# RemcoHoger/Space-Filling-Curves-for-Vision-Transformers

Hardware: AMD Instinct MI355X
Metric: images/sec ViT-B/16 224px Hilbert-order training (higher is better)
Workload: dtype bf16; 1 GPU; vit_b16_224_hilbert: 224x224 Hilbert pixel order, 16x16-pixel tokens, batch 256/GPU, full train step (fwd+CE+bwd+clip+AdamW); global_batch=256, parallelism=dp1, hip_graph=False

## Files before the change

### space-filling-curves-for-vision-transformers_amd/csrc/gemm8p.hip

```cpp
#include "common_host.h"
#include "gemm_core.h"
#include <mutex>
#include <type_traits>
#include <unordered_map>

namespace sfcvit {
namespace {

using namespace gemm_core;

namespace p8 {

constexpr int T = 512, HALF = 16384, KTB = 65536, LDS_BYTES = 2 * KTB;
constexpr int LDS_TQ = LDS_BYTES, LDS_PATCH = LDS_TQ + 64, LDS_BIAS = LDS_PATCH + 8 * 2048, LDS_MAX = P8_LDS_MAX;
static_assert(LDS_BIAS == P8_LDS_BIAS, "dispatch.h prices the bias vector at this offset");
enum { RELU = P8_RELU, DROP = P8_DROP, RES = P8_RES, DACT = P8_DACT, CSUM = P8_CSUM, BITS = P8_BITS };

typedef const __attribute__((address_space(1))) void *gptr_t;
typedef __attribute__((address_space(3))) void *lptr_t;

template <int N> __device__ __forceinline__ void wait_vm() { asm volatile("s_waitcnt vmcnt(%0)" ::"n"(N) : "memory"); }
template <int N> __device__ __forceinline__ void wait_lgkm() {
    asm volatile("s_waitcnt lgkmcnt(%0)" ::"n"(N) : "memory");
    __builtin_amdgcn_sched_barrier(0);
}
__device__ __forceinline__ void bar() {
    __builtin_amdgcn_sched_barrier(0);
    __builtin_amdgcn_s_barrier();
    __builtin_amdgcn_sched_barrier(0);
}

struct Cursor {
    int tile, k0;
    const uint16_t *p;
};

struct StoreMap {
    int wa;
    int ra;
    long coff;
};

template <int MASK>
__device__ __forceinline__ void epilogue_math(const sfcvit_gemm_args &g, int m, int n, float (&v)[16], const float (&bv)[16],
                                              const u32x4 (&side)[2], uint32_t thresh, float keep_scale, float dact_scale,
                                              uint32_t rk_in0, uint32_t rk_in1, u32x4 &w0, u32x4 &w1) {
    if (!(MASK & DACT)) {
#pragma unroll
        for (int r = 0; r < 16; r++) v[r] += bv[r];
    }
    if (MASK & RELU) {
#pragma unroll
        for (int r = 0; r < 16; r++) v[r] = fmaxf(v[r], 0.f);
    }
    if (MASK & DROP) {
        const uint64_t row = uint64_t(m) + uint64_t(uint32_t(g.row_offset));
        const uint32_t rk = mix32(uint32_t(row) * 0x9E3779B1u + ((row >> 32) ? rk_in1 : rk_in0));
#pragma unroll
        for (int p = 0; p < 8; p++) {
            bool k0, k1;
            drop_keep2(rk, uint32_t(n >> 1) + p, thresh, k0, k1);
            v[2 * p] = k0 ? v[2 * p] * keep_scale : 0.f;
            v[2 * p + 1] = k1 ? v[2 * p + 1] * keep_scale : 0.f;
        }
    }
    if (MASK & RES) {
        float rv[16];
        unpack8f(side[0], rv);
        unpack8f(side[1], rv + 8);
#pragma unroll
        for (int r = 0; r < 16; r++) v[r] += rv[r];
    }
    if ((MASK & BITS) && (MASK & RELU)) {
        uint32_t bits = 0;
#pragma unroll
        for (int r = 0; r < 16; r++) bits |= uint32_t(v[r] > 0.f) << r;
        uint8_t *mp = static_cast<uint8_t *>(g.actmask) + size_t(m) * g.ld_actmask + (n >> 3);
        asm volatile("global_store_short %0, %1, off\n\ts_nop 1" ::"v"(mp), "v"(bits) : "memory");
    }
    if (MASK & DACT) {
        if (MASK & BITS) {
            const uint32_t bits = side[0][0];
#pragma unroll
            for (int r = 0; r < 16; r++) v[r] = (bits >> r & 1u) ? v[r] * dact_scale : 0.f;
        } else {
            float a[16];
            unpack8f(side[0], a);
            unpack8f(side[1], a + 8);
#pragma unroll
            for (int r = 0; r < 16; r++) v[r] = a[r] > 0.f ? v[r] * dact_scale : 0.f;
        }
    }
    w0 = u32x4{pack2bf(v[0], v[1]), pack2bf(v[2], v[3]), pack2bf(v[4], v[5]), pack2bf(v[6], v[7])};
    w1 = u32x4{pack2bf(v[8], v[9]), pack2bf(v[10], v[11]), pack2bf(v[12], v[13]), pack2bf(v[14], v[15])};
}

#define SFCVIT_XROW(a, b) "ds_write_b128 %[wa], " a "\n\tds_write_b128 %[wb], " b "\n\tds_read_b128 " a ", %[ra]\n\tds_read_b128 " b ", %[ra] offset:1024\n\t"
template <int NR>
__device__ __forceinline__ void patch_exchange(u32x4 (&w)[NR][2], const StoreMap &sm) {
    static_assert(NR >= 1 && NR <= 8, "rows per batch");
    const int wa = sm.wa, wb = sm.wa ^ 16, ra = sm.ra;
    if constexpr (NR == 8)
        asm volatile(SFCVIT_XROW("%0", "%1") SFCVIT_XROW("%2", "%3") SFCVIT_XROW("%4", "%5") SFCVIT_XROW("%6", "%7")
                     SFCVIT_XROW("%8", "%9") SFCVIT_XROW("%10", "%11") SFCVIT_XROW("%12", "%13") SFCVIT_XROW("%14", "%15") "s_waitcnt lgkmcnt(0)"
                     : "+v"(w[0][0]), "+v"(w[0][1]), "+v"(w[1][0]), "+v"(w[1][1]), "+v"(w[2][0]), "+v"(w[2][1]), "+v"(w[3][0]), "+v"(w[3][1]),
                       "+v"(w[4][0]), "+v"(w[4][1]), "+v"(w[5][0]), "+v"(w[5][1]), "+v"(w[6][0]), "+v"(w[6][1]), "+v"(w[7][0]), "+v"(w[7][1])
                     : [wa] "v"(wa), [wb] "v"(wb), [ra] "v"(ra) : "memory");
    else if constexpr (NR == 7)
        asm volatile(SFCVIT_XROW("%0", "%1") SFCVIT_XROW("%2", "%3") SFCVIT_XROW("%4", "%5") SFCVIT_XROW("%6", "%7")
                     SFCVIT_XROW("%8", "%9") SFCVIT_XROW("%10", "%11") SFCVIT_XROW("%12", "%13") "s_waitcnt lgkmcnt(0)"
                     : "+v"(w[0][0]), "+v"(w[0][1]), "+v"(w[1][0]), "+v"(w[1][1]), "+v"(w[2][0]), "+v"(w[2][1]), "+v"(w[3][0]), "+v"(w[3][1]),
                       "+v"(w[4][0]), "+v"(w[4][1]), "+v"(w[5][0]), "+v"(w[5][1]), "+v"(w[6][0]), "+v"(w[6][1])
                     : [wa] "v"(wa), [wb] "v"(wb), [ra] "v"(ra) : "memory");
    else if constexpr (NR == 6)
        asm volatile(SFCVIT_XROW("%0", "%1") SFCVIT_XROW("%2", "%3") SFCVIT_XROW("%4", "%5") SFCVIT_XROW("%6", "%7")
                     SFCVIT_XROW("%8", "%9") SFCVIT_XROW("%10", "%11") "s_waitcnt lgkmcnt(0)"
                     : "+v"(w[0][0]), "+v"(w[0][1]), "+v"(w[1][0]), "+v"(w[1][1]), "+v"(w[2][0]), "+v"(w[2][1]), "+v"(w[3][0]), "+v"(w[3][1]),
                       "+v"(w[4][0]), "+v"(w[4][1]), "+v"(w[5][0]), "+v"(w[5][1])
                     : [wa] "v"(wa), [wb] "v"(wb), [ra] "v"(ra) : "memory");
    else if constexpr (NR == 4)
        asm volatile(SFCVIT_XROW("%0", "%1") SFCVIT_XROW("%2", "%3") SFCVIT_XROW("%4", "%5") SFCVIT_XROW("%6", "%7") "s_waitcnt lgkmcnt(0)"
                     : "+v"(w[0][0]), "+v"(w[0][1]), "+v"(w[1][0]), "+v"(w[1][1]), "+v"(w[2][0]), "+v"(w[2][1]), "+v"(w[3][0]), "+v"(w[3][1])
                     : [wa] "v"(wa), [wb] "v"(wb), [ra] "v"(ra) : "memory");
    else
        static_assert(NR == 8, "patch_exchange: batch sizes 4, 6, 7, 8");
}
#undef SFCVIT_XROW

__device__ __forceinline__ void store_row_pair(const sfcvit_gemm_args &g, int m, int n, const StoreMap &sm, const u32x4 &w0, const u32x4 &w1) {
    uint16_t *c = static_cast<uint16_t *>(g.c) + size_t(m) * g.ldc + n + sm.coff;
    asm volatile("global_store_dwordx4 %0, %1, off sc0 sc1 nt\n\ts_nop 1" ::"v"(c), "v"(w0) : "memory");
    asm volatile("global_store_dwordx4 %0, %1, off sc0 sc1 nt\n\ts_nop 1" ::"v"(c + size_t(8) * g.ldc), "v"(w1) : "memory");
}


template <int NI, int MASK, bool P2 = false>
__global__ __launch_bounds__(T) void gemm8p_kernel(const sfcvit_gemm_args g, unsigned *__restrict__ counters, int stag_slots, int stag_ticks, int walk) {
    constexpr int BM = 32 * NI, GR = 16 * NI;
    extern __shared__ __attribute__((aligned(16))) char smem[];
    if (stag_ticks > 0) {
        const uint64_t until = __builtin_amdgcn_s_memrealtime() + uint64_t((blockIdx.x >> 3) % stag_slots) * uint64_t(stag_ticks);
        while (__builtin_amdgcn_s_memrealtime() < until) __builtin_amdgcn_s_sleep(8);
    }
    const int tid = threadIdx.x, lane = tid & 63, wid = __builtin_amdgcn_readfirstlane(tid >> 6), wr = wid >> 2, wc = wid & 3;
    const int q = lane >> 4, nl = lane & 15;
    const int K = g.K, NT = g.N / 256, ntiles = ((g.M + BM - 1) / BM) * NT, KT = K / 64, m_last = g.M - BM;
    const uint16_t *A = static_cast<const uint16_t *>(g.a);
    const uint16_t *B = static_cast<const uint16_t *>(g.b);
    const int G = gridDim.x, per_xcd = G >> 3, xcd = blockIdx.x & 7;
    int *const tq = reinterpret_cast<int *>(smem + LDS_TQ);
    auto tile_of = [&](unsigned l) __attribute__((always_inline)) {
        const long t = long(l / unsigned(per_xcd)) * G + xcd * per_xcd + int(l % unsigned(per_xcd));
        if (t >= ntiles) return -1;
        if (walk > 0 && walk < NT) {
            const unsigned MT = unsigned(ntiles / NT), full = unsigned(NT / walk) * MT * unsigned(walk), ut = unsigned(t);
            const unsigned wcur = ut < full ? unsigned(walk) : unsigned(NT % walk), base = ut < full ? (ut / (MT * walk)) * walk : unsigned(NT / walk) * walk;
            const unsigned tt = ut < full ? ut % (MT * walk) : ut - full;
            return int((tt / wcur) << 16 | (base + tt % wcur));
        }
        return int((unsigned(t) / unsigned(NT)) << 16 | (unsigned(t) % unsigned(NT)));
    };
    auto finish = [&]() __attribute__((always_inline)) {
        if (tid == 0) {
            const unsigned old = atomicAdd(counters + 8, 1u);
            if (old == unsigned(G) - 1u) {
#pragma unroll
                for (int i = 0; i < 9; i++) counters[i] = 0u;
            }
        }
    };
    if (tid == 0) {
        const unsigned l0 = atomicAdd(counters + xcd, 1u);
        tq[0] = tile_of(l0);
        const unsigned l1 = atomicAdd(counters + xcd, 1u);
        tq[1] = tile_of(l1);
    }
    const bool has_bias = !(MASK & DACT) && g.bias != nullptr;
    if (has_bias)
        for (int i = tid; i < g.N / 8; i += T)
            *reinterpret_cast<u32x4 *>(smem + LDS_BIAS + i * 16) = static_cast<const u32x4 *>(g.bias)[i];
    __syncthreads();

    int tile_cur = __builtin_amdgcn_readfirstlane(tq[0]);
    if (tile_cur < 0) { finish(); return; }
    unsigned drawn = 0;
    if (tid == 0) drawn = atomicAdd(counters + xcd, 1u);
    const int tile_first = tile_cur;
    int t = 0;

    const int r1 = 8 * wid + (lane >> 3);
    const int sc = (lane & 7) ^ ((r1 >> 1) & 7);
    const int w1 = (r1 < GR - 64) ? r1 : r1 - (NI == 7 ? 16 : 32);
    const int b_row = (r1 >> 5) * 64 + ((r1 & 15) >> 2) * 16 + ((r1 >> 4) & 1) * 4 + (r1 & 3);
    const uint32_t voffA0 = (uint32_t(r1) * uint32_t(g.lda) + sc * 8) * 2, voffA1 = (uint32_t(64 + w1) * uint32_t(g.lda) + sc * 8) * 2;
    const uint32_t voffB = (uint32_t(b_row) * uint32_t(g.ldb) + sc * 8) * 2;
    const size_t a_second = size_t(GR) * g.lda, b_second = size_t(128) * g.ldb, b_h1 = size_t(8) * g.ldb;

    auto cursor_at = [&](int seq, int tile, bool is_a) __attribute__((always_inline)) {
        Cursor c;
        c.tile = seq;
        c.k0 = 0;
        if (tile < 0) tile = tile_first;
        c.p = is_a ? A + size_t(min((tile >> 16) * BM, m_last)) * g.lda : B + size_t(tile & 0xFFFF) * 256 * g.ldb;
        return c;
    };
    const uint16_t *next_a = nullptr, *next_b = nullptr;
    auto set_next = [&](int seq) __attribute__((always_inline)) {
        const Cursor na = cursor_at(seq, __builtin_amdgcn_readfirstlane(tq[seq & 3]), true);
        const Cursor nb = cursor_at(seq, __builtin_amdgcn_readfirstlane(tq[seq & 3]), false);
        next_a = na.p;
        next_b = nb.p;
    };
    auto advance = [&](Cursor &c, bool is_a) __attribute__((always_inline)) {
        if (c.k0 + 64 == K) { c.tile++; c.k0 = 0; c.p = is_a ? next_a : next_b; }
        else { c.k0 += 64; c.p += 64; }
    };
    const int m0_wave = wid * 1024;
    auto dma16 = [&](const uint16_t *base, uint32_t voff, int lds) __attribute__((always_inline)) {
        asm volatile("s_mov_b32 m0, %2\n\ts_nop 0\n\tglobal_load_lds_dwordx4 %0, %1"
                     :
                     : "v"(voff), "s"(base), "s"(lds)
                     : "memory");
    };
    auto stage_a = [&](const Cursor &c, int buf, int h) __attribute__((always_inline)) {
        const int d = m0_wave + buf * KTB + h * HALF;
        const uint32_t vo = h ? voffA1 : voffA0;
        dma16(c.p, vo, d);
        dma16(c.p + a_second, vo, d + 8192);
    };
    auto stage_b = [&](const Cursor &c, int buf, int h) __attribute__((always_inline)) {
        const uint16_t *p = c.p + (h ? b_h1 : 0);
        const int d = m0_wave + buf * KTB + 2 * HALF + h * HALF;
        dma16(p, voffB, d);
        dma16(p + b_second, voffB, d + 8192);
    };

    const int o0 = nl * 128 + ((q ^ ((nl >> 1) & 7)) << 4);
    const int a_off0 = wr * 8192 + o0, a_off1 = wr * 8192 + (o0 ^ 64);
    const int b_off0 = 2 * HALF + wc * 4096 + o0, b_off1 = 2 * HALF + wc * 4096 + (o0 ^ 64);
    bf16x8 fa0[4][2], fa1[NI - 4][2], fb0[2][2], fb1[2][2];
    auto read_a0 = [&](int buf) __attribute__((always_inline)) {
#pragma unroll
        for (int i = 0; i < 4; i++) {
            fa0[i][0] = *reinterpret_cast<const bf16x8 *>(smem + a_off0 + buf * KTB + i * 2048);
            fa0[i][1] = *reinterpret_cast<const bf16x8 *>(smem + a_off1 + buf * KTB + i * 2048);
        }
    };
    auto read_a1 = [&](int buf) __attribute__((always_inline)) {
#pragma unroll
        for (int i = 0; i < NI - 4; i++) {
            fa1[i][0] = *reinterpret_cast<const bf16x8 *>(smem + a_off0 + buf * KTB + HALF + i * 2048);
            fa1[i][1] = *reinterpret_cast<const bf16x8 *>(smem + a_off1 + buf * KTB + HALF + i * 2048);
        }
    };
    auto read_b = [&](bf16x8 (&fb)[2][2], int buf, int sub) __attribute__((always_inline)) {
#pragma unroll
        for (int j = 0; j < 2; j++) {
            fb[j][0] = *reinterpret_cast<const bf16x8 *>(smem + b_off0 + buf * KTB + sub * HALF + j * 2048);
            fb[j][1] = *reinterpret_cast<const bf16x8 *>(smem + b_off1 + buf * KTB + sub * HALF + j * 2048);
        }
    };

    f32x4 acc[NI][4];
    auto zero_acc = [&]() __attribute__((always_inline)) {
#pragma unroll
        for (int i = 0; i < NI; i++)
#pragma unroll
            for (int j = 0; j < 4; j++) acc[i][j] = f32x4{0.f, 0.f, 0.f, 0.f};
    };
    auto mma0 = [&](const bf16x8 (&fb)[2][2], int bsub) __attribute__((always_inline)) {
        __builtin_amdgcn_s_setprio(1);
#pragma unroll
        for (int kk = 0; kk < 2; kk++)
#pragma unroll
            for (int i = 0; i < 4; i++)
#pragma unroll
                for (int j = 0; j < 2; j++)
                    acc[i][bsub * 2 + j] = __builtin_amdgcn_mfma_f32_16x16x32_bf16(fb[j][kk], fa0[i][kk], acc[i][bsub * 2 + j], 0, 0, 0);
        __builtin_amdgcn_s_setprio(0);
    };
    auto mma1 = [&](const bf16x8 (&fb)[2][2], int bsub) __attribute__((always_inline)) {
        __builtin_amdgcn_s_setprio(1);
#pragma unroll
        for (int kk = 0; kk < 2; kk++)
#pragma unroll
            for (int i = 0; i < NI - 4; i++)
#pragma unroll
                for (int j = 0; j < 2; j++)
                    acc[4 + i][bsub * 2 + j] = __builtin_amdgcn_mfma_f32_16x16x32_bf16(fb[j][kk], fa1[i][kk], acc[4 + i][bsub * 2 + j], 0, 0, 0);
        __builtin_amdgcn_s_setprio(0);
    };

    const uint32_t thresh = (MASK & DROP) ? drop_thresh(g.dropout_p) : 0u;
    const float keep_scale = (MASK & DROP) ? 1.f / (1.f - g.dropout_p) : 1.f;
    const uint32_t seed_e = (MASK & DROP) ? eff_seed(g.dropout_seed, g.seed_off) : 0u;
    const uint32_t rk_in0 = (MASK & DROP) ? mix32(seed_e) : 0u, rk_in1 = (MASK & DROP) ? mix32(seed_e ^ 0x7FEB352Du) : 0u;
    const float dact_scale = g.dact_scale != 0.f ? g.dact_scale : 1.f;
    auto draw = [&]() __attribute__((always_inline)) {
        if (tid == 0) {
            tq[(t + 2) & 3] = tile_of(drawn);
            drawn = atomicAdd(counters + xcd, 1u);
        }
    };
    auto epilogue = [&]() __attribute__((always_inline)) {
        const int tile = tile_cur;
        int te = tid;
        asm volatile("" : "+v"(te));
        const int le = te & 63, qe = le >> 4, ne = le & 15;
        StoreMap sm;
        {
            const int patch = LDS_PATCH + wid * 2048, r0 = le >> 3, ch = le & 7;
            sm.wa = patch + ne * 128 + (((2 * qe) ^ (ne & 7)) << 4);
            sm.ra = patch + r0 * 128 + ((ch ^ r0) << 4);
            sm.coff = long(r0 - ne) * g.ldc + (8 * ch - 16 * qe);
        }
        const int m_new = (tile >> 16) * BM;
        const int m0 = min(m_new, m_last) + wr * GR + ne, n0 = (tile & 0xFFFF) * 256 + wc * 64 + qe * 16;
        mfma_fence();
        float bv[16];
        if (has_bias) {
            const char *bp = smem + LDS_BIAS + n0 * 2;
            unpack8f(*reinterpret_cast<const u32x4 *>(bp), bv);
            unpack8f(*reinterpret_cast<const u32x4 *>(bp + 16), bv + 8);
        } else {
#pragma unroll
            for (int r = 0; r < 16; r++) bv[r] = 0.f;
        }
        const uint16_t *sp = (MASK & RES) ? static_cast<const uint16_t *>(g.residual) : static_cast<const uint16_t *>(g.aux_in);
        const size_t ld_side = (MASK & RES) ? size_t(g.ldr) : size_t(g.ldaux);
        float cs[16];
#pragma unroll
        for (int r = 0; r < 16; r++) cs[r] = 0.f;
        auto batch = [&](auto i0c, auto i1c) __attribute__((always_inline)) {
            constexpr int i0 = decltype(i0c)::value, i1 = decltype(i1c)::value;
            u32x4 side[i1 - i0][2];
            if ((MASK & DACT) && (MASK & BITS)) {
#pragma unroll
                for (int i = i0; i < i1; i++)
                    side[i - i0][0][0] = *reinterpret_cast<const uint16_t *>(static_cast<const uint8_t *>(g.actmask) +
                                                                             size_t(m0 + 16 * i) * g.ld_actmask + (n0 >> 3));
            } else if (MASK & (RES | DACT)) {
#pragma unroll
                for (int i = i0; i < i1; i++) {
                    const uint16_t *p = sp + size_t(m0 + 16 * i) * ld_side + n0;
                    side[i - i0][0] = *reinterpret_cast<const u32x4 *>(p);
                    side[i - i0][1] = *reinterpret_cast<const u32x4 *>(p + 8);
                }
            }
            u32x4 pk[i1 - i0][2];
            static_for<i0, i1>([&](auto ic) __attribute__((always_inline)) {
                constexpr int i = decltype(ic)::value;
                float v[16] = {acc[i][0][0], acc[i][0][1], acc[i][0][2], acc[i][0][3], acc[i][1][0], acc[i][1][1],
                               acc[i][1][2], acc[i][1][3], acc[i][2][0], acc[i][2][1], acc[i][2][2], acc[i][2][3],
                               acc[i][3][0], acc[i][3][1], acc[i][3][2], acc[i][3][3]};
                epilogue_math<MASK>(g, m0 + 16 * i, n0, v, bv, side[i - i0], thresh, keep_scale, dact_scale, rk_in0, rk_in1,
                                    pk[i - i0][0], pk[i - i0][1]);
                if (MASK & CSUM) {
                    const bool own = m0 + 16 * i >= m_new;
#pragma unroll
                    for (int r = 0; r < 16; r++) cs[r] += own ? v[r] : 0.f;
                }
            });
            patch_exchange<i1 - i0>(pk, sm);
            static_for<i0, i1>([&](auto ic) __attribute__((always_inline)) {
                constexpr int i = decltype(ic)::value;
                store_row_pair(g, m0 + 16 * i, n0, sm, pk[i - i0][0], pk[i - i0][1]);
            });
        };
        if constexpr (NI == 8 && ((MASK & (DROP | RES)) == (DROP | RES) || (MASK & (DACT | CSUM | BITS)) == (DACT | CSUM))) {
            batch(std::integral_constant<int, 0>{}, std::integral_constant<int, 4>{});
            batch(std::integral_constant<int, 4>{}, std::integral_constant<int, NI>{});
        } else {
            batch(std::integral_constant<int, 0>{}, std::integral_constant<int, NI>{});
        }
        if (MASK & CSUM) {
#pragma unroll
            for (int r = 0; r < 16; r++) cs[r] = row16_sum(cs[r]);
            if (ne == 0) {
                float *pp = static_cast<float *>(g.workspace) + size_t(2 * (tile >> 16) + wr) * g.N + n0;
#pragma unroll
                for (int r4 = 0; r4 < 4; r4++)
                    *reinterpret_cast<f32x4 *>(pp + 4 * r4) = f32x4{cs[4 * r4], cs[4 * r4 + 1], cs[4 * r4 + 2], cs[4 * r4 + 3]};
            }
        }
        zero_acc();
    };

    Cursor ca = cursor_at(0, tile_cur, true), cb = cursor_at(0, tile_cur, false);
    stage_b(cb, 0, 0); stage_a(ca, 0, 0); stage_a(ca, 0, 1); stage_b(cb, 0, 1);
    advance(ca, true);
    advance(cb, false);
    if (P2) {
        stage_b(cb, 1, 0); stage_a(ca, 1, 0); stage_b(cb, 1, 1);
        advance(cb, false);
        wait_vm<6>();
    } else {
        stage_b(cb, 1, 0); stage_a(ca, 1, 0); stage_a(ca, 1, 1); stage_b(cb, 1, 1);
        advance(ca, true);
        advance(cb, false);
        wait_vm<8>();
    }
    bar();
    if (wr == 1) bar();
    zero_acc();

    constexpr int NSTORE = 2 * NI + ((MASK & CSUM) ? 4 : 0) + (((MASK & BITS) && (MASK & RELU)) ? NI : 0);
    auto stage_next = [&](int buf) __attribute__((always_inline)) {
        stage_a(ca, buf, 1);
        advance(ca, true);
        stage_b(cb, buf, 1);
        advance(cb, false);
        __builtin_amdgcn_sched_barrier(0);
    };
    auto ktile = [&](int buf, bool first, bool last) __attribute__((always_inline)) {
        read_b(fb0, buf, 0);
        read_a0(buf);
        bar();
        wait_lgkm<0>();
        mma0(fb0, 0);
        bar();
        read_a1(buf);
        bar();
        wait_lgkm<0>();
        mma1(fb0, 0);
        if (first) set_next(t + 1);
        bar();
        read_b(fb1, buf, 1);
        stage_b(cb, buf, 0);
        bar();
        wait_lgkm<0>();
        mma1(fb1, 1);
        bar();
        stage_a(ca, buf, 0);
        if (first && t > 0) wait_vm<4 + NSTORE>();
        else wait_vm<4>();
        bar();
        mma0(fb1, 1);
        if (last) {
            if (wr == 0) {
                bar();
                draw();
            }
            stage_next(buf);
            epilogue();
            if (wr == 1) bar();
        } else {
            bar();
            stage_next(buf);
        }
    };
    auto ktile2 = [&](int buf, bool first, bool last) __attribute__((always_inline)) {
        read_b(fb0, buf, 0);
        read_b(fb1, buf, 1);
        read_a0(buf);
        stage_a(ca, buf ^ 1, 1);
        advance(ca, true);
        __builtin_amdgcn_sched_barrier(0);
        if (first && t > 0) wait_vm<8 + NSTORE>();
        else wait_vm<8>();
        wait_lgkm<0>();
        bar();
        mma0(fb0, 0);
        mma0(fb1, 1);
        if (first) set_next(t + 1);
        bar();
        read_a1(buf);
        stage_b(cb, buf, 0);
        stage_a(ca, buf, 0);
        stage_b(cb, buf, 1);
        advance(cb, false);
        __builtin_amdgcn_sched_barrier(0);
        if (first && t > 0) wait_vm<8 + NSTORE>();
        else wait_vm<8>();
        wait_lgkm<0>();
        bar();
        mma1(fb0, 0);
        mma1(fb1, 1);
        if (last) {
            if (wr == 0) {
                bar();
                draw();
            }
            epilogue();
            if (wr == 1) bar();
        } else {
            bar();
        }
    };
    int kt = 0;
    for (;;) {
        if (P2) ktile2(0, kt == 0, false);
        else ktile(0, kt == 0, false);
        kt += 2;
        const bool last = kt == KT;
        if (P2) ktile2(1, false, last);
        else ktile(1, false, last);
        if (last) {
            kt = 0;
            t++;
            tile_cur = __builtin_amdgcn_readfirstlane(tq[t & 3]);
            if (tile_cur < 0) break;
        }
    }
    if (wr == 0) bar();
    wait_vm<0>();
    finish();
}


template <bool P2>
__global__ __launch_bounds__(T) void gemm8p_km_kernel(const sfcvit_gemm_args g, int kt_per_split, int nsplits) {
    extern __shared__ __attribute__((aligned(16))) char smem[];
    const int tid = threadIdx.x, lane = tid & 63, wid = tid >> 6, wr = wid >> 2, wc = wid & 3;
    const int q4 = lane >> 4, nl = lane & 15;
    const int NT = g.N / 256, KT = g.K / 64;
    const int tiles = (g.M / 256) * NT;
    const int unit = (blockIdx.x & 7) * (gridDim.x >> 3) + (blockIdx.x >> 3);
    if (unit >= tiles * nsplits) return;
    const int tile = unit % tiles, z = unit / tiles;
    const int m0 = (tile / NT) * 256, n0 = (tile % NT) * 256;
    const int kt_beg = z * kt_per_split;
    const int nkt = min(kt_per_split, KT - kt_beg);
    const uint16_t *A = static_cast<const uint16_t *>(g.a) + size_t(kt_beg) * 64 * g.lda + m0;
    const uint16_t *B = static_cast<const uint16_t *>(g.b) + size_t(kt_beg) * 64 * g.ldb + n0;

    const int kr = 4 * wid + (lane >> 4);
    const int sw = (kr & 3) | (((kr >> 3) & 1) << 2);
    const int c16 = ((((lane & 15) >> 1) ^ sw) << 1) | (lane & 1);
    const size_t offA = size_t(kr) * g.lda + c16 * 8, offB = size_t(kr) * g.ldb + c16 * 8;
    const size_t a32 = size_t(32) * g.lda, b32 = size_t(32) * g.ldb, a64 = size_t(64) * g.lda, b64 = size_t(64) * g.ldb;
    char *const lds_piece = smem + tid * 16;
    const uint16_t *ca = A, *cb = B;
    int akt = 0, bkt = 0;
    auto advance_a = [&]() __attribute__((always_inline)) {
        if (++akt < nkt) ca += a64;
    };
    auto advance_b = [&]() __attribute__((always_inline)) {
        if (++bkt < nkt) cb += b64;
    };
    auto stage_a = [&](int buf, int h) __attribute__((always_inline)) {
        const uint16_t *p = ca + offA + h * 128;
        char *d = lds_piece + buf * KTB + h * HALF;
        __builtin_amdgcn_global_load_lds((gptr_t)p, (lptr_t)d, 16, 0, 0);
        __builtin_amdgcn_global_load_lds((gptr_t)(p + a32), (lptr_t)(d + 8192), 16, 0, 0);
    };
    auto stage_b = [&](int buf, int h) __attribute__((always_inline)) {
        const uint16_t *p = cb + offB + h * 128;
        char *d = lds_piece + buf * KTB + 2 * HALF + h * HALF;
        __builtin_amdgcn_global_load_lds((gptr_t)p, (lptr_t)d, 16, 0, 0);
        __builtin_amdgcn_global_load_lds((gptr_t)(p + b32), (lptr_t)(d + 8192), 16, 0, 0);
    };

    const int qq = nl >> 2, pp = nl & 3;
    const int lane_sw = qq | ((q4 & 1) << 2);
    const int row_off = (8 * q4 + qq) * 256 + 8 * pp;
    int a_addr[8], b_addr[4];
#pragma unroll
    for (int i = 0; i < 8; i++)
        a_addr[i] = (i >> 2) * HALF + row_off + (((wr * 4 + (i & 3)) ^ lane_sw) << 5);
#pragma unroll
    for (int j = 0; j < 4; j++)
        b_addr[j] = 2 * HALF + (j >> 1) * HALF + row_off + (((wc * 2 + (j & 1)) ^ lane_sw) << 5);
#define SFCVIT_TR(dst, addr, off) asm volatile("ds_read_b64_tr_b16 %0, %1 offset:" #off : "=v"(dst) : "v"(addr) : "memory")
    auto tr_frag2 = [&](bf16x8 (&f)[2], int addr) __attribute__((always_inline)) {
        bf16x4 l0, h0, l1, h1;
        SFCVIT_TR(l0, addr, 0);
        SFCVIT_TR(h0, addr, 1024);
        SFCVIT_TR(l1, addr, 8192);
        SFCVIT_TR(h1, addr, 9216);
        f[0] = __builtin_shufflevector(l0, h0, 0, 1, 2, 3, 4, 5, 6, 7);
        f[1] = __builtin_shufflevector(l1, h1, 0, 1, 2, 3, 4, 5, 6, 7);
    };
    bf16x8 fa0[4][2], fa1[4][2], fb0[2][2], fb1[2][2];
    auto read_a2 = [&](bf16x8 (&fa)[4][2], int sub, int i0) __attribute__((always_inline)) {
#pragma unroll
        for (int i = i0; i < i0 + 2; i++) tr_frag2(fa[i], a_addr[sub * 4 + i]);
    };
    auto read_b = [&](bf16x8 (&fb)[2][2], int sub) __attribute__((always_inline)) {
#pragma unroll
        for (int j = 0; j < 2; j++) tr_frag2(fb[j], b_addr[sub * 2 + j]);
    };
    auto flip = [&]() __attribute__((always_inline)) {
#pragma unroll
        for (int i = 0; i < 8; i++) a_addr[i] ^= KTB;
#pragma unroll
        for (int j = 0; j < 4; j++) b_addr[j] ^= KTB;
    };

    f32x4 acc[8][4];
#pragma unroll
    for (int i = 0; i < 8; i++)
#pragma unroll
        for (int j = 0; j < 4; j++) acc[i][j] = f32x4{0.f, 0.f, 0.f, 0.f};
    auto mma = [&](const bf16x8 (&fa)[4][2], const bf16x8 (&fb)[2][2], int asub, int bsub) __attribute__((always_inline)) {
        __builtin_amdgcn_s_setprio(1);
#pragma unroll
        for (int kk = 0; kk < 2; kk++)
#pragma unroll
            for (int i = 0; i < 4; i++)
#pragma unroll
                for (int j = 0; j < 2; j++)
                    acc[asub * 4 + i][bsub * 2 + j] =
                        __builtin_amdgcn_mfma_f32_16x16x32_bf16(fb[j][kk], fa[i][kk], acc[asub * 4 + i][bsub * 2 + j], 0, 0, 0);
        __builtin_amdgcn_s_setprio(0);
    };

    if (P2) {
        stage_b(0, 0); stage_a(0, 0); stage_a(0, 1); stage_b(0, 1);
        advance_a();
        advance_b();
        stage_b(1, 0); stage_a(1, 0); stage_b(1, 1);
        advance_b();
        wait_vm<6>();
        bar();
        if (wr == 1) bar();
        auto ktile2 = [&](int buf) __attribute__((always_inline)) {
            read_b(fb0, 0);
            read_b(fb1, 1);
            read_a2(fa0, 0, 0);
            read_a2(fa0, 0, 2);
            stage_a(buf ^ 1, 1);
            advance_a();
            wait_vm<8>();
            wait_lgkm<0>();
            bar();
            mma(fa0, fb0, 0, 0);
            mma(fa0, fb1, 0, 1);
            bar();
            read_a2(fa1, 1, 0);
            read_a2(fa1, 1, 2);
            stage_b(buf, 0);
            stage_a(buf, 0);
            stage_b(buf, 1);
            advance_b();
            wait_vm<8>();
            wait_lgkm<0>();
            bar();
            mma(fa1, fb0, 1, 0);
            mma(fa1, fb1, 1, 1);
            bar();
            flip();
        };
        for (int k = 0; k < nkt; k += 2) {
            ktile2(0);
            ktile2(1);
        }
    } else {
        stage_b(0, 0); stage_a(0, 0); stage_a(0, 1); stage_b(0, 1);
        advance_a();
        advance_b();
        stage_b(1, 0); stage_a(1, 0);
        wait_vm<4>();
        bar();
        if (wr == 1) bar();
        auto ktile = [&](int buf) __attribute__((always_inline)) {
            read_b(fb0, 0);
            read_a2(fa0, 0, 0);
            read_a2(fa0, 0, 2);
            stage_a(buf ^ 1, 1);
            advance_a();
            bar();
            wait_lgkm<0>();
            mma(fa0, fb0, 0, 0);
            bar();
            read_a2(fa1, 1, 0);
            read_a2(fa1, 1, 2);
            stage_b(buf ^ 1, 1);
            advance_b();
            bar();
            wait_lgkm<0>();
            mma(fa1, fb0, 1, 0);
            bar();
            read_b(fb1, 1);
            stage_b(buf, 0);
            bar();
            wait_lgkm<0>();
            mma(fa1, fb1, 1, 1);
            bar();
            stage_a(buf, 0);
            wait_vm<4>();
            bar();
            mma(fa0, fb1, 0, 1);
            bar();
            flip();
        };
        for (int k = 0; k < nkt; k += 2) {
            ktile(0);
            ktile(1);
        }
}
    if (wr == 0) bar();
    wait_vm<0>();
    mfma_fence();
    float *slab = static_cast<float *>(g.workspace) + size_t(z) * g.M * g.N + size_t(m0 + wr * 64 + nl) * g.N + n0 + wc * 32 + 4 * q4;
#pragma unroll
    for (int i = 0; i < 8; i++)
#pragma unroll
        for (int j = 0; j < 4; j++)
            *reinterpret_cast<f32x4 *>(slab + size_t((i >> 2) * 128 + (i & 3) * 16) * g.N + (j >> 1) * 128 + (j & 1) * 16) = acc[i][j];
}

struct DeviceState {
    unsigned *pool = nullptr;
    int next = 0;
    std::unordered_map<hipStream_t, unsigned *> per_stream;
};
constexpr int MAX_DEVICES = 64, SLOTS = 1024, SLOT_UINTS = 16;
std::mutex g_mu;
DeviceState g_dev[MAX_DEVICES];

unsigned *queue_counters(hipStream_t s) {
    std::lock_guard<std::mutex> lock(g_mu);
    int dev = 0;
    if (hipGetDevice(&dev) != hipSuccess || dev < 0 || dev >= MAX_DEVICES) return nullptr;
    DeviceState *d = &g_dev[dev];
    auto it = d->per_stream.find(s);
    if (it != d->per_stream.end()) return it->second;
    if (!d->pool) {
        if (hipMalloc(reinterpret_cast<void **>(&d->pool), size_t(SLOTS) * SLOT_UINTS * sizeof(unsigned)) != hipSuccess ||
            hipMemset(d->pool, 0, size_t(SLOTS) * SLOT_UINTS * sizeof(unsigned)) != hipSuccess) {
            d->pool = nullptr;
            return nullptr;
        }
    }
    if (d->next >= SLOTS) return nullptr;
    unsigned *p = d->pool + size_t(d->next++) * SLOT_UINTS;
    d->per_stream[s] = p;
    return p;
}

template <int NI, int MASK>
int launch(const GemmPlan &p, const sfcvit_gemm_args &a, unsigned *counters, hipStream_t s) {
    const int LDS_TOTAL = LDS_BIAS + (a.bias ? a.N * 2 : 0);
    if (p.p2) {
        if (int rc = raise_lds_limit(reinterpret_cast<const void *>(&gemm8p_kernel<NI, MASK, true>), LDS_MAX, "gemm8p attribute")) return rc;
        hipLaunchKernelGGL((gemm8p_kernel<NI, MASK, true>), dim3(p.grid), dim3(T), LDS_TOTAL, s, a, counters, p.stag_slots, p.stag_ticks, p.walk);
    } else {
        if (int rc = raise_lds_limit(reinterpret_cast<const void *>(&gemm8p_kernel<NI, MASK>), LDS_MAX, "gemm8p attribute")) return rc;
        hipLaunchKernelGGL((gemm8p_kernel<NI, MASK>), dim3(p.grid), dim3(T), LDS_TOTAL, s, a, counters, p.stag_slots, p.stag_ticks, p.walk);
    }
    const int rc = check_launch("gemm8p");
    if (rc) (void)hipMemsetAsync(counters, 0, SLOT_UINTS * sizeof(unsigned), s);
    return rc;
}

template <int NI>
int launch_mask(const GemmPlan &p, const sfcvit_gemm_args &a, unsigned *counters, hipStream_t s) {
    switch (p.mask) {
    case 0: return launch<NI, 0>(p, a, counters, s);
    case RES: return launch<NI, RES>(p, a, counters, s);
    case DROP | RES: return launch<NI, DROP | RES>(p, a, counters, s);
    case RELU: return launch<NI, RELU>(p, a, counters, s);
    case RELU | DROP: return launch<NI, RELU | DROP>(p, a, counters, s);
    case DACT: return launch<NI, DACT>(p, a, counters, s);
    case DACT | CSUM: return launch<NI, DACT | CSUM>(p, a, counters, s);
    case RELU | BITS: return launch<NI, RELU | BITS>(p, a, counters, s);
    case RELU | DROP | BITS: return launch<NI, RELU | DROP | BITS>(p, a, counters, s);
    case DACT | BITS: return launch<NI, DACT | BITS>(p, a, counters, s);
    case DACT | CSUM | BITS: return launch<NI, DACT | CSUM | BITS>(p, a, counters, s);
    default: return fail(SFCVIT_EINVAL, "gemm8p: no kernel for epilogue mask %d", p.mask);
    }
}

}
}

unsigned *stream_counters(void *stream) { return p8::queue_counters(static_cast<hipStream_t>(stream)); }

int gemm8p_launch(const GemmPlan &p, const sfcvit_gemm_args &a, hipStream_t s) {
    using namespace p8;
    unsigned *counters = queue_counters(s);
    if (!counters) return fail(SFCVIT_ELAUNCH, "gemm8p: could not allocate the tile-queue counters");
    if (p.ni == 8) return launch_mask<8>(p, a, counters, s);
    if (p.ni == 7) return launch_mask<7>(p, a, counters, s);
    return launch_mask<6>(p, a, counters, s);
}

int gemm8p_km_launch(const GemmPlan &p, const sfcvit_gemm_args &a, hipStream_t s) {
    using namespace p8;
    sfcvit_gemm_args body = a;
    body.K = p.k_done;
    if (p.p2) {
        if (int rc = raise_lds_limit(reinterpret_cast<const void *>(&gemm8p_km_kernel<true>), LDS_BYTES, "gemm8p_km attribute")) return rc;
        hipLaunchKernelGGL(gemm8p_km_kernel<true>, dim3(p.grid), dim3(T), LDS_BYTES, s, body, p.k_per_split, p.splits);
    } else {
        if (int rc = raise_lds_limit(reinterpret_cast<const void *>(&gemm8p_km_kernel<false>), LDS_BYTES, "gemm8p_km attribute")) return rc;
        hipLaunchKernelGGL(gemm8p_km_kernel<false>, dim3(p.grid), dim3(T), LDS_BYTES, s, body, p.k_per_split, p.splits);
    }
    return check_launch("gemm8p_km");
}

}
```

Measured before the change: 8294 images/s.

## Cut epilogue register pressure by re-reading kernel args and packing float math

Epilogue scalar arguments (pointers, strides, dropout params) are now re-read from the kernarg segment inside the epilogue and tile-draw paths for masked variants, so those values need not stay live in SGPRs/VGPRs across the main loop. Bias add and column-sum accumulation use packed two-wide float vectors. Relu mask bit packing becomes an inline-asm compare/add-with-carry chain, and the backward relu masking uses bitfield-extract AND instead of selects. Together these aim to shorten the epilogue and reduce register pressure, at the cost of extra scalar loads and brittle inline assembly.

```diff
diff --git a/space-filling-curves-for-vision-transformers_amd/csrc/gemm8p.hip b/space-filling-curves-for-vision-transformers_amd/csrc/gemm8p.hip
--- a/space-filling-curves-for-vision-transformers_amd/csrc/gemm8p.hip
+++ b/space-filling-curves-for-vision-transformers_amd/csrc/gemm8p.hip
@@ -18,6 +18,14 @@
 
 typedef const __attribute__((address_space(1))) void *gptr_t;
 typedef __attribute__((address_space(3))) void *lptr_t;
+struct KernArgs {
+    sfcvit_gemm_args g;
+    unsigned *counters;
+    int stag_slots, stag_ticks, walk;
+};
+typedef const __attribute__((address_space(4))) KernArgs *kargs_t;
+static_assert(sizeof(sfcvit_gemm_args) % 8 == 0 && offsetof(KernArgs, counters) == sizeof(sfcvit_gemm_args), "KernArgs mirrors the parameter list");
+typedef __attribute__((ext_vector_type(2))) float f32x2;
 
 template <int N> __device__ __forceinline__ void wait_vm() { asm volatile("s_waitcnt vmcnt(%0)" ::"n"(N) : "memory"); }
 template <int N> __device__ __forceinline__ void wait_lgkm() {
@@ -46,8 +54,17 @@
                                               const u32x4 (&side)[2], uint32_t thresh, float keep_scale, float dact_scale,
                                               uint32_t rk_in0, uint32_t rk_in1, u32x4 &w0, u32x4 &w1) {
     if (!(MASK & DACT)) {
-#pragma unroll
-        for (int r = 0; r < 16; r++) v[r] += bv[r];
+        if (MASK & RELU) {
+#pragma unroll
+            for (int p = 0; p < 8; p++) {
+                const f32x2 s = f32x2{v[2 * p], v[2 * p + 1]} + f32x2{bv[2 * p], bv[2 * p + 1]};
+                v[2 * p] = s[0];
+                v[2 * p + 1] = s[1];
+            }
+        } else {
+#pragma unroll
+            for (int r = 0; r < 16; r++) v[r] += bv[r];
+        }
     }
     if (MASK & RELU) {
 #pragma unroll
@@ -73,16 +90,35 @@
     }
     if ((MASK & BITS) && (MASK & RELU)) {
         uint32_t bits = 0;
-#pragma unroll
-        for (int r = 0; r < 16; r++) bits |= uint32_t(v[r] > 0.f) << r;
+        uint64_t c0, c1, c2;
+#define SFCVIT_CMP(c, x) "v_cmp_lt_f32_e64 " c ", 0, " x "\n\t"
+#define SFCVIT_ADC(c) "v_addc_co_u32_e64 %[b], vcc, %[b], %[b], " c "\n\t"
+        asm(SFCVIT_CMP("%[c0]", "%[v15]") SFCVIT_CMP("%[c1]", "%[v14]") SFCVIT_CMP("%[c2]", "%[v13]")
+            SFCVIT_ADC("%[c0]") SFCVIT_CMP("%[c0]", "%[v12]") SFCVIT_ADC("%[c1]") SFCVIT_CMP("%[c1]", "%[v11]")
+            SFCVIT_ADC("%[c2]") SFCVIT_CMP("%[c2]", "%[v10]") SFCVIT_ADC("%[c0]") SFCVIT_CMP("%[c0]", "%[v9]")
+            SFCVIT_ADC("%[c1]") SFCVIT_CMP("%[c1]", "%[v8]") SFCVIT_ADC("%[c2]") SFCVIT_CMP("%[c2]", "%[v7]")
+            SFCVIT_ADC("%[c0]") SFCVIT_CMP("%[c0]", "%[v6]") SFCVIT_ADC("%[c1]") SFCVIT_CMP("%[c1]", "%[v5]")
+            SFCVIT_ADC("%[c2]") SFCVIT_CMP("%[c2]", "%[v4]") SFCVIT_ADC("%[c0]") SFCVIT_CMP("%[c0]", "%[v3]")
+            SFCVIT_ADC("%[c1]") SFCVIT_CMP("%[c1]", "%[v2]") SFCVIT_ADC("%[c2]") SFCVIT_CMP("%[c2]", "%[v1]")
+            SFCVIT_ADC("%[c0]") SFCVIT_CMP("%[c0]", "%[v0]") SFCVIT_ADC("%[c1]") SFCVIT_ADC("%[c2]") SFCVIT_ADC("%[c0]")
+            : [b] "+v"(bits), [c0] "=&s"(c0), [c1] "=&s"(c1), [c2] "=&s"(c2)
+            : [v0] "v"(v[0]), [v1] "v"(v[1]), [v2] "v"(v[2]), [v3] "v"(v[3]), [v4] "v"(v[4]), [v5] "v"(v[5]), [v6] "v"(v[6]),
+              [v7] "v"(v[7]), [v8] "v"(v[8]), [v9] "v"(v[9]), [v10] "v"(v[10]), [v11] "v"(v[11]), [v12] "v"(v[12]),
+              [v13] "v"(v[13]), [v14] "v"(v[14]), [v15] "v"(v[15])
+            : "vcc");
+#undef SFCVIT_CMP
+#undef SFCVIT_ADC
         uint8_t *mp = static_cast<uint8_t *>(g.actmask) + size_t(m) * g.ld_actmask + (n >> 3);
         asm volatile("global_store_short %0, %1, off\n\ts_nop 1" ::"v"(mp), "v"(bits) : "memory");
     }
     if (MASK & DACT) {
         if (MASK & BITS) {
             const uint32_t bits = side[0][0];
-#pragma unroll
-            for (int r = 0; r < 16; r++) v[r] = (bits >> r & 1u) ? v[r] * dact_scale : 0.f;
+            static_for<0, 16>([&](auto rc) __attribute__((always_inline)) {
+                uint32_t on;
+                asm("v_bfe_i32 %0, %1, %2, 1" : "=v"(on) : "v"(bits), "n"(decltype(rc)::value));
+                v[decltype(rc)::value] = __uint_as_float(__float_as_uint(v[decltype(rc)::value] * dact_scale) & on);
+            });
         } else {
             float a[16];
             unpack8f(side[0], a);
@@ -134,6 +170,18 @@
 }
 
 
+__device__ __forceinline__ int tile_at(unsigned l, int per_xcd, int G, int xcd, int ntiles, int NT, int walk) {
+    const long t = long(l / unsigned(per_xcd)) * G + xcd * per_xcd + int(l % unsigned(per_xcd));
+    if (t >= ntiles) return -1;
+    if (walk > 0 && walk < NT) {
+        const unsigned MT = unsigned(ntiles / NT), full = unsigned(NT / walk) * MT * unsigned(walk), ut = unsigned(t);
+        const unsigned wcur = ut < full ? unsigned(walk) : unsigned(NT % walk), base = ut < full ? (ut / (MT * walk)) * walk : unsigned(NT / walk) * walk;
+        const unsigned tt = ut < full ? ut % (MT * walk) : ut - full;
+        return int((tt / wcur) << 16 | (base + tt % wcur));
+    }
+    return int((unsigned(t) / unsigned(NT)) << 16 | (unsigned(t) % unsigned(NT)));
+}
+
 template <int NI, int MASK, bool P2 = false>
 __global__ __launch_bounds__(T) void gemm8p_kernel(const sfcvit_gemm_args g, unsigned *__restrict__ counters, int stag_slots, int stag_ticks, int walk) {
     constexpr int BM = 32 * NI, GR = 16 * NI;
@@ -160,12 +208,26 @@
         }
         return int((unsigned(t) / unsigned(NT)) << 16 | (unsigned(t) % unsigned(NT)));
     };
+    auto kargs_again = [&]() __attribute__((always_inline)) {
+        kargs_t kp = (kargs_t)__builtin_amdgcn_kernarg_segment_ptr();
+        asm volatile("" : "+s"(kp));
+        return kp;
+    };
     auto finish = [&]() __attribute__((always_inline)) {
         if (tid == 0) {
-            const unsigned old = atomicAdd(counters + 8, 1u);
-            if (old == unsigned(G) - 1u) {
-#pragma unroll
-                for (int i = 0; i < 9; i++) counters[i] = 0u;
+            if constexpr ((MASK & DROP) != 0) {
+                unsigned *cn = kargs_again()->counters;
+                const unsigned old = atomicAdd(cn + 8, 1u);
+                if (old == unsigned(G) - 1u) {
+#pragma unroll
+                    for (int i = 0; i < 9; i++) cn[i] = 0u;
+                }
+            } else {
+                const unsigned old = atomicAdd(counters + 8, 1u);
+                if (old == unsigned(G) - 1u) {
+#pragma unroll
+                    for (int i = 0; i < 9; i++) counters[i] = 0u;
+                }
             }
         }
     };
@@ -175,8 +237,8 @@
         const unsigned l1 = atomicAdd(counters + xcd, 1u);
         tq[1] = tile_of(l1);
     }
-    const bool has_bias = !(MASK & DACT) && g.bias != nullptr;
-    if (has_bias)
+    const bool has_bias_0 = !(MASK & DACT) && g.bias != nullptr;
+    if (has_bias_0)
         for (int i = tid; i < g.N / 8; i += T)
             *reinterpret_cast<u32x4 *>(smem + LDS_BIAS + i * 16) = static_cast<const u32x4 *>(g.bias)[i];
     __syncthreads();
@@ -291,19 +353,35 @@
         __builtin_amdgcn_s_setprio(0);
     };
 
-    const uint32_t thresh = (MASK & DROP) ? drop_thresh(g.dropout_p) : 0u;
-    const float keep_scale = (MASK & DROP) ? 1.f / (1.f - g.dropout_p) : 1.f;
-    const uint32_t seed_e = (MASK & DROP) ? eff_seed(g.dropout_seed, g.seed_off) : 0u;
-    const uint32_t rk_in0 = (MASK & DROP) ? mix32(seed_e) : 0u, rk_in1 = (MASK & DROP) ? mix32(seed_e ^ 0x7FEB352Du) : 0u;
-    const float dact_scale = g.dact_scale != 0.f ? g.dact_scale : 1.f;
     auto draw = [&]() __attribute__((always_inline)) {
         if (tid == 0) {
-            tq[(t + 2) & 3] = tile_of(drawn);
-            drawn = atomicAdd(counters + xcd, 1u);
+            if constexpr (MASK & DROP) {
+                const kargs_t kp = kargs_again();
+                const int NTd = kp->g.N / 256;
+                tq[(t + 2) & 3] = tile_at(drawn, per_xcd, G, xcd, ((kp->g.M + BM - 1) / BM) * NTd, NTd, kp->walk);
+                drawn = atomicAdd(kp->counters + xcd, 1u);
+            } else {
+                tq[(t + 2) & 3] = tile_of(drawn);
+                drawn = atomicAdd(counters + xcd, 1u);
+            }
         }
     };
     auto epilogue = [&]() __attribute__((always_inline)) {
         const int tile = tile_cur;
+        sfcvit_gemm_args ge = g;
+        if constexpr (MASK != 0) {
+            const kargs_t kp = kargs_again();
+            ge.c = kp->g.c; ge.ldc = kp->g.ldc; ge.N = kp->g.N; ge.bias = kp->g.bias; ge.workspace = kp->g.workspace;
+            ge.residual = kp->g.residual; ge.ldr = kp->g.ldr; ge.aux_in = kp->g.aux_in; ge.ldaux = kp->g.ldaux;
+            ge.actmask = kp->g.actmask; ge.ld_actmask = kp->g.ld_actmask; ge.row_offset = kp->g.row_offset;
+            ge.dropout_p = kp->g.dropout_p; ge.dropout_seed = kp->g.dropout_seed; ge.seed_off = kp->g.seed_off; ge.dact_scale = kp->g.dact_scale;
+        }
+        const bool has_bias = MASK != 0 ? !(MASK & DACT) && ge.bias != nullptr : has_bias_0;
+        const uint32_t thresh = (MASK & DROP) ? drop_thresh(ge.dropout_p) : 0u;
+        const float keep_scale = (MASK & DROP) ? 1.f / (1.f - ge.dropout_p) : 1.f;
+        const uint32_t seed_e = (MASK & DROP) ? eff_seed(ge.dropout_seed, ge.seed_off) : 0u;
+        const uint32_t rk_in0 = (MASK & DROP) ? mix32(seed_e) : 0u, rk_in1 = (MASK & DROP) ? mix32(seed_e ^ 0x7FEB352Du) : 0u;
+        const float dact_scale = ge.dact_scale != 0.f ? ge.dact_scale : 1.f;
         int te = tid;
         asm volatile("" : "+v"(te));
         const int le = te & 63, qe = le >> 4, ne = le & 15;
@@ -312,7 +390,7 @@
             const int patch = LDS_PATCH + wid * 2048, r0 = le >> 3, ch = le & 7;
             sm.wa = patch + ne * 128 + (((2 * qe) ^ (ne & 7)) << 4);
             sm.ra = patch + r0 * 128 + ((ch ^ r0) << 4);
-            sm.coff = long(r0 - ne) * g.ldc + (8 * ch - 16 * qe);
+            sm.coff = long(r0 - ne) * ge.ldc + (8 * ch - 16 * qe);
         }
         const int m_new = (tile >> 16) * BM;
         const int m0 = min(m_new, m_last) + wr * GR + ne, n0 = (tile & 0xFFFF) * 256 + wc * 64 + qe * 16;
@@ -326,19 +404,19 @@
 #pragma unroll
             for (int r = 0; r < 16; r++) bv[r] = 0.f;
         }
-        const uint16_t *sp = (MASK & RES) ? static_cast<const uint16_t *>(g.residual) : static_cast<const uint16_t *>(g.aux_in);
-        const size_t ld_side = (MASK & RES) ? size_t(g.ldr) : size_t(g.ldaux);
-        float cs[16];
-#pragma unroll
-        for (int r = 0; r < 16; r++) cs[r] = 0.f;
+        const uint16_t *sp = (MASK & RES) ? static_cast<const uint16_t *>(ge.residual) : static_cast<const uint16_t *>(ge.aux_in);
+        const size_t ld_side = (MASK & RES) ? size_t(ge.ldr) : size_t(ge.ldaux);
+        f32x2 cs[8];
+#pragma unroll
+        for (int p = 0; p < 8; p++) cs[p] = f32x2{0.f, 0.f};
         auto batch = [&](auto i0c, auto i1c) __attribute__((always_inline)) {
             constexpr int i0 = decltype(i0c)::value, i1 = decltype(i1c)::value;
             u32x4 side[i1 - i0][2];
             if ((MASK & DACT) && (MASK & BITS)) {
 #pragma unroll
                 for (int i = i0; i < i1; i++)
-                    side[i - i0][0][0] = *reinterpret_cast<const uint16_t *>(static_cast<const uint8_t *>(g.actmask) +
-                                                                             size_t(m0 + 16 * i) * g.ld_actmask + (n0 >> 3));
+                    side[i - i0][0][0] = *reinterpret_cast<const uint16_t *>(static_cast<const uint8_t *>(ge.actmask) +
+                                                                             size_t(m0 + 16 * i) * ge.ld_actmask + (n0 >> 3));
             } else if (MASK & (RES | DACT)) {
 #pragma unroll
                 for (int i = i0; i < i1; i++) {
@@ -348,23 +426,27 @@
                 }
             }
             u32x4 pk[i1 - i0][2];
+            int nb = n0;
+            if constexpr (NI == 8 && (MASK & (DROP | RES)) == (DROP | RES)) asm volatile("" : "+v"(nb));
             static_for<i0, i1>([&](auto ic) __attribute__((always_inline)) {
                 constexpr int i = decltype(ic)::value;
                 float v[16] = {acc[i][0][0], acc[i][0][1], acc[i][0][2], acc[i][0][3], acc[i][1][0], acc[i][1][1],
                                acc[i][1][2], acc[i][1][3], acc[i][2][0], acc[i][2][1], acc[i][2][2], acc[i][2][3],
                                acc[i][3][0], acc[i][3][1], acc[i][3][2], acc[i][3][3]};
-                epilogue_math<MASK>(g, m0 + 16 * i, n0, v, bv, side[i - i0], thresh, keep_scale, dact_scale, rk_in0, rk_in1,
+                epilogue_math<MASK>(ge, m0 + 16 * i, nb, v, bv, side[i - i0], thresh, keep_scale, dact_scale, rk_in0, rk_in1,
                                     pk[i - i0][0], pk[i - i0][1]);
                 if (MASK & CSUM) {
-                    const bool own = m0 + 16 * i >= m_new;
-#pragma unroll
-                    for (int r = 0; r < 16; r++) cs[r] += own ? v[r] : 0.f;
+                    if (m_new <= m_last || m0 + 16 * i >= m_new) {
+                        asm volatile("");
+#pragma unroll
+                        for (int p = 0; p < 8; p++) cs[p] += f32x2{v[2 * p], v[2 * p + 1]};
+                    }
                 }
             });
             patch_exchange<i1 - i0>(pk, sm);
             static_for<i0, i1>([&](auto ic) __attribute__((always_inline)) {
                 constexpr int i = decltype(ic)::value;
-                store_row_pair(g, m0 + 16 * i, n0, sm, pk[i - i0][0], pk[i - i0][1]);
+                store_row_pair(ge, m0 + 16 * i, n0, sm, pk[i - i0][0], pk[i - i0][1]);
             });
         };
         if constexpr (NI == 8 && ((MASK & (DROP | RES)) == (DROP | RES) || (MASK & (DACT | CSUM | BITS)) == (DACT | CSUM))) {
@@ -375,12 +457,19 @@
         }
         if (MASK & CSUM) {
 #pragma unroll
-            for (int r = 0; r < 16; r++) cs[r] = row16_sum(cs[r]);
+            for (int p = 0; p < 8; p++) {
+                float lo = cs[p][0], hi = cs[p][1];
+                asm("" : "+v"(lo), "+v"(hi));
+                lo = row16_sum(lo);
+                hi = row16_sum(hi);
+                asm("" : "+v"(lo), "+v"(hi));
+                cs[p] = f32x2{lo, hi};
+            }
             if (ne == 0) {
-                float *pp = static_cast<float *>(g.workspace) + size_t(2 * (tile >> 16) + wr) * g.N + n0;
+                float *pp = static_cast<float *>(ge.workspace) + size_t(2 * (tile >> 16) + wr) * ge.N + n0;
 #pragma unroll
                 for (int r4 = 0; r4 < 4; r4++)
-                    *reinterpret_cast<f32x4 *>(pp + 4 * r4) = f32x4{cs[4 * r4], cs[4 * r4 + 1], cs[4 * r4 + 2], cs[4 * r4 + 3]};
+                    *reinterpret_cast<f32x4 *>(pp + 4 * r4) = f32x4{cs[2 * r4][0], cs[2 * r4][1], cs[2 * r4 + 1][0], cs[2 * r4 + 1][1]};
             }
         }
         zero_acc();
```

After: 8327 images/s (median of 2 runs). Within noise of the previous version (+0.4%).
